# Nuos/jpgEnc

Hardware: AMD Instinct MI355X
Metric: MPixels/s encode (4K 4:2:0 Q=90) (higher is better)
Workload: dtype f64; 1 GPU; 3840x2160 4:2:0 Q90 full encode (RGB8 in HBM -> .jpg bytes in HBM), 3072 frames per GPU per step over 32 distinct inputs; width=3840, height=2160, quality=90, subsampling=4:2:0, distinct_inputs_per_gpu=32, parallelism=frames sharded over 1 GPU(s), no data-path collective, avg_jpeg_bytes=4581380

## Files before the change

jpgenc_amd/csrc/encoder.cpp:

```cpp
#include "encoder_impl.hpp"
#include "host_par.hpp"

#include <algorithm>
#include <array>
#include <condition_variable>
#include <cstdlib>
#include <cstdio>
#include <mutex>
#include <string>
#include <thread>

#include <sys/prctl.h>
#include <vector>

namespace jpge {

hipError_t wait_event(hipEvent_t e) {
    hipError_t r;
    while ((r = hipEventQuery(e)) == hipErrorNotReady) {
    }
    return r;
}
int wait_seq(const uint64_t* word, uint64_t seq, hipStream_t stream, int nap_us, const std::atomic<int>* queued,
             WaitGuess* guess, const std::function<bool()>* work) {
// ... 289 lines not shown
    if (mode) *mode = huff_mode_;
    if (specs && huff_mode_)
        for (int t = 0; t < 4; ++t) specs[t] = huff_specs_[t];
}

int Encoder::fixed_tables(Slot& s, bool& fresh) {
    const bool gray = s.g.gray();
    Slot::FixedKey k;
    k.gen = huff_gen_;
    k.w = s.img_w;
    k.h = s.img_h;
    k.restart = s.rst.mcus;
    k.samp = gray ? 0u : (s.g.yh << 4) | s.g.yv();
    std::memcpy(k.qy, s.qy, 64);
    std::memcpy(k.qc, s.qc, 64);
    s.symbols = 0;
    fresh = !(k == s.fixed);
    if (fresh) {
        s.fixed.gen = 0;
        std::memcpy(s.h_tab, huff_words_, kTabBytes);
        if (gray) std::memset(s.h_tab + 2 * 256, 0, 2 * 256 * sizeof(uint32_t));
        const HuffTable* tp[4] = {&huff_tabs_[0], &huff_tabs_[1], &huff_tabs_[2], &huff_tabs_[3]};
        const std::vector<uint8_t> hdr = gray ? jfif_headers_gray(s.img_w, s.img_h, s.qy, tp, s.rst.mcus)
                                              : jfif_headers(s.img_w, s.img_h, s.qy, s.qc, tp, s.rst.mcus,
                                                             (uint8_t)k.samp);
        if (hdr.size() > kHdrMax) return kErrInternal;
        std::memcpy(reinterpret_cast<uint8_t*>(s.h_tab) + kTabBytes, hdr.data(), hdr.size());
        s.hdr_len = hdr.size();
        s.fixed = k;
    }
    if (s.out_cap && s.out_cap < s.hdr_len + 2) return kErrNoSpace;
    return kOk;
}

size_t Encoder::max_jpeg_bytes(uint32_t w, uint32_t h) {
    size_t cap = 0;
    for (int mode : {420, 444, 422, 411}) {
        const Geometry g = geometry(w, h, mode);
        cap = std::max(cap, 2048 + (size_t)g.nblocks() * 2 * 209 + 16 + (size_t)g.nmcu() * 4);
    }
    return cap;
}

int Encoder::open(int device, std::unique_ptr<Encoder>& out, int lanes) {
    int n = 0;
    if (hipGetDeviceCount(&n) != hipSuccess || n <= 0) return kErrNoDevice;
    if (device < 0 || device >= n) return kErrNoDevice;
    JPGE_HIP(hipSetDevice(device));
    std::unique_ptr<Encoder> e(new Encoder());
    e->device_ = device;
    if (const char* ew = std::getenv("JPGE_ENTROPY_WGS")) e->entropy_wgs_ = (uint32_t)std::strtoul(ew, nullptr, 10);
    if (const char* sw = std::getenv("JPGE_STATS_WGS")) e->stats_wgs_ = (uint32_t)std::strtoul(sw, nullptr, 10);
    e->fdct_wgs_ = (uint32_t)env_int("JPGE_FDCT_WGS", 0, 0, 65536);
    e->stamps_file_ = std::getenv("JPGE_STAMPS_FILE");
    e->host_trace_file_ = std::getenv("JPGE_HOST_TRACE");
    e->cpu_prof_ = env_int("JPGE_CPU_PROF", 0, 0, 1) != 0;
    e->lat_prof_ = env_int("JPGE_LAT_PROF", 0, 0, 1) != 0;
    e->table_helper_ = env_int("JPGE_TABLE_HELPER", 1, 0, 1) != 0;
    e->gate_ = env_int("JPGE_GATE", 1, 0, 2);
    if (env_int("AMD_SERIALIZE_KERNEL", 0, 0, 3) != 0 || env_int("HIP_LAUNCH_BLOCKING", 0, 0, 1) != 0) e->gate_ = 0;
    if (const int us = env_int("JPGE_TEST_GATE_TIMEOUT_US", 0, 0, 1000000)) e->gate_ticks_ = 100ull * (uint64_t)us;
    e->gate_delay_us_ = env_int("JPGE_TEST_GATE_DELAY_US", 0, 0, 1000000);
    if (e->gate_ == 2) {
        int wv = 0;
        if (hipDeviceGetAttribute(&wv, hipDeviceAttributeCanUseStreamWaitValue, device) != hipSuccess || !wv) e->gate_ = 0;
        (void)hipGetLastError();
    }
    e->hist_nap_us_ = env_int("JPGE_HIST_NAP_US", e->hist_nap_us_, 0, 1000);
    e->lookahead_ = env_int("JPGE_LOOKAHEAD", e->lookahead_, 1, kMaxLookahead);
    e->drain_lag_ = env_int("JPGE_DRAIN_LAG", e->drain_lag_, 0, kMaxDrainLag);
    e->set_ = env_int("JPGE_SET", 0, 0, kMaxSet);
    e->nap_us_ = env_int("JPGE_NAP_US", e->nap_us_, 1, 1000);
    e->first_sleep_ = env_int("JPGE_FIRST_SLEEP", (int)(e->first_sleep_ * 100 + 0.5), 0, 95) / 100.0;
    const int nap = env_int("JPGE_NAP", -1, -1, 1);
    e->ext_place_ = env_int("JPGE_EXT_PLACE", -1, -1, 1);
    e->place_in_code_ = env_int("JPGE_PLACE_IN_CODE", 1, 0, 1) != 0;
    if (e->stamps_file_) {
        e->dbg_words_ = 4ull * 65536 * kStampSlots;
        JPGE_HIP(hipMalloc((void**)&e->d_dbg_, e->dbg_words_ * 8));
        JPGE_HIP(hipMemset(e->d_dbg_, 0, e->dbg_words_ * 8));
    }
    const int nlanes = e->stamps_file_ ? 1
                       : lanes > 0   ? std::min(lanes, kMaxLanes)
                                     : env_int("JPGE_LANES", 4, 1, kMaxLanes);
    e->nap_ = nap < 0 ? nlanes > 1 : nap != 0;
    const int nslots = e->lookahead_ + e->drain_lag_ + 1;
    const bool cumask = env_int("JPGE_CU_MASK_STREAMS", nlanes > 1 ? 1 : 0, 0, 1) != 0;
    std::vector<uint32_t> mask;
    if (cumask) {
        int ncu = 0;
        JPGE_HIP(hipDeviceGetAttribute(&ncu, hipDeviceAttributeMultiprocessorCount, device));
        mask.assign((size_t)(ncu + 31) / 32, 0xFFFFFFFFu);
        if (ncu % 32) mask.back() = (1u << (ncu % 32)) - 1u;
    }
    for (int l = 0; l < nlanes; ++l) {
        std::unique_ptr<Lane> ln(new Lane());
        ln->id = l;
        if (!cumask || hipExtStreamCreateWithCUMask(&ln->stream, (uint32_t)mask.size(), mask.data()) != hipSuccess) {
            (void)hipGetLastError();
            JPGE_HIP(hipStreamCreateWithFlags(&ln->stream, hipStreamNonBlocking));
        }
        JPGE_HIP(hipEventCreateWithFlags(&ln->done, hipEventDisableTiming));
        ln->guess_hist.frac = ln->guess_result.frac = e->first_sleep_;
        if (const int st = e->add_slots(*ln, nslots)) return st;
        if (l > 0) ln->start();
        e->lanes_.push_back(std::move(ln));
// ... 143 lines not shown
    a.imp_dst = imp ? reinterpret_cast<uint4*>(imp->d_tab) : nullptr;
    a.imp_n16 = imp ? (uint32_t)((kTabBytes + imp->hdr_len + 15) / 16) : 0u;
    a.dbg = d_dbg_;
    return a;
}

StatsArgs Encoder::stats_args(Slot& s) {
    const CtlLayout L(slot_layout(s).grid());
    StatsArgs st;
    st.coef = s.d_coef;
    st.g = s.g;
    st.hist.cnt = reinterpret_cast<uint32_t*>(s.d_ctl + L.cnt);
    st.hist.key = reinterpret_cast<uint64_t*>(s.d_ctl + L.key);
    st.seed = s.seed;
    st.rst = s.rst;
    st.key_y0 = s.key_y0;
    st.key_c0 = s.key_c0;
    st.key_ncb = s.key_ncb;
    st.seg = seg_layout(s.g, s.rst.mcus, entropy_wgs());
    st.recs = s.d_recs;
    st.tcount = s.d_tcount;
    st.wgs = stats_wgs();
    if (!stats_wgs_ && lanes_.size() > 1) {
        const uint32_t t = seg_tiles(st.seg);
        if (t < 3u * 384u) st.wgs = std::max(1u, (t + 2) / 3);
    }
    st.dbg = d_dbg_ ? d_dbg_ + 65536 * kStampSlots : nullptr;
    return st;
}

EntropyArgs Encoder::entropy_args(Slot& s) {
    const CtlLayout L(slot_layout(s).grid());
    EntropyArgs e;
    e.coef = s.d_coef;
    e.recs = s.d_recs;
    e.tcount = s.d_tcount;
    e.g = s.g;
    e.tables = s.d_tab;
    e.out = s.out_dev;
    e.hdr_len = s.hdr_len;
    e.out_cap = s.out_cap;
    e.rec = s.d_ctl + L.rec;
    e.place = reinterpret_cast<WgPlace*>(s.d_ctl + L.place);
    e.summary = reinterpret_cast<StripeSummary*>(s.d_ctl + L.summary);
    if (ext_place_ > 0 || (ext_place_ < 0 && lanes_.size() > 1)) {
        e.flags |= kExtPlace;
        if (place_in_code_ && !s.rst.mcus && slot_layout(s).grid() <= kPlaceInCodeMaxWgs)
            e.done = reinterpret_cast<uint32_t*>(s.d_ctl + L.done);
    }
    e.host_result = s.d_result_host;
    e.seq = s.seq;
    e.ubuf = s.d_ubuf;
    e.wgs = entropy_wgs_;
    e.seed = s.seed;
    e.rst = s.rst;
    e.seg = slot_layout(s);
    if (s.rst.mcus) {
        e.seg_index0 = s.rst.mcu0 / s.rst.mcus;
        e.seg_markers0 = e.seg_index0 > 0 ? 1u : 0u;
    }
    Slot::carry_export(e, nullptr);
    e.dbg = d_dbg_ ? d_dbg_ + 2 * 65536 * kStampSlots : nullptr;
    return e;
}

int Encoder::prep1(Slot& s, const FrameDesc& f, const uint8_t qy[64], const uint8_t qc[64], uint32_t flags,
                   Slot* imp, FdctArgs& a, StatsArgs& st) {
    if (!f.rgb || f.width == 0 || f.height == 0 || f.width > 65535 || f.height > 65535) return kErrArg;
    if (f.maxval < 1 || f.maxval > 255) return kErrRange;
    const bool gray = fmt_gray(f.fmt);
    const Geometry g = gray ? gray_geometry(f.width, f.height) : geometry(f.width, f.height, mode_);
    if (!fmt_valid(f.fmt) || (f.plane_stride && fmt_planes(f.fmt) == 1)) return kErrArg;
    if (fmt_yuv(f.fmt) && (f.maxval != 255 || (fmt_yuv420(f.fmt) && mode_ != 420))) return kErrArg;
    if (gray && f.maxval != 255) return kErrArg;
    if (fmt_yuv10(f.fmt) && (((uintptr_t)f.rgb | f.stride | f.plane_stride) & 1)) return kErrArg;
    if (gray) qc = qy;
    const size_t row = (size_t)fmt_row_bytes(f.fmt, f.width);
    const size_t stride = f.stride ? f.stride : row;
    if (stride < row) return kErrArg;
    const size_t planes = fmt_planes(f.fmt);
    const size_t plane_stride = f.plane_stride ? f.plane_stride : stride * f.height;
    const bool half = fmt_yuv420(f.fmt) || f.fmt == kFmtI422;
    const size_t dev_pitch = align_up(row, f.fmt == kFmtI420 || f.fmt == kFmtI422 || f.fmt == kFmtI010 ? 32 : 16);
    const size_t dev_plane = dev_pitch * f.height;
    const size_t crows = f.fmt == kFmtI422 ? f.height : chroma_dim(f.height),
                 crow = f.fmt == kFmtNv12 || f.fmt == kFmtP010 ? row : (size_t)fmt_bpp(f.fmt) * chroma_dim(f.width);
    const size_t cpitch = (size_t)fmt_chroma_pitch(f.fmt, stride), dev_cpitch = (size_t)fmt_chroma_pitch(f.fmt, dev_pitch);
    const size_t dev_bytes = half ? dev_plane + (planes - 1) * dev_cpitch * crows : planes * dev_plane;
    const bool dev_in = (flags & kFlagDeviceInput) != 0, dev_out = (flags & kFlagDeviceOutput) != 0;
    if (!k1_offsets_fit(f.fmt, g, dev_in ? stride : dev_pitch)) return kErrArg;
    const size_t in_bytes = dev_in ? 0 : dev_bytes;
    const size_t out_cap = dev_out ? 0 : max_jpeg_bytes(f.width, f.height);
    if (!tables_nonzero(qy, qc)) return kErrArg;
    const int st0 = ensure(s, g, in_bytes, out_cap);
    if (st0) return st0;
    if (!dev_in) {
        if (stride == dev_pitch && (planes == 1 || plane_stride == dev_plane))
            JPGE_HIP(hipMemcpyAsync(s.d_in, f.rgb, dev_bytes, hipMemcpyHostToDevice, s.stream));
        else if (half) {
            JPGE_HIP(hipMemcpy2DAsync(s.d_in, dev_pitch, f.rgb, stride, (size_t)fmt_bpp(f.fmt) * f.width, f.height, hipMemcpyHostToDevice,
                                      s.stream));
            for (size_t c = 0; c + 1 < planes; ++c)
                JPGE_HIP(hipMemcpy2DAsync(s.d_in + dev_plane + c * dev_cpitch * crows, dev_cpitch,
                                          f.rgb + plane_stride + c * cpitch * crows, cpitch, crow, crows,
                                          hipMemcpyHostToDevice, s.stream));
        } else
// ... 655 lines not shown
```

jpgenc_amd/csrc/encoder.hpp:

```cpp
#pragma once
#include <atomic>
#include <chrono>
#include <cstddef>
#include <cstdint>
#include <memory>
#include <functional>
#include <mutex>
#include <vector>

#include <hip/hip_runtime_api.h>

#include "host_io.hpp"
#include "huffman.hpp"
#include "kernels.hpp"
#include "planes.hpp"

namespace jpge {

constexpr uint32_t kFlagDeviceInput = 1u;
constexpr uint32_t kFlagDeviceOutput = 2u;
constexpr uint32_t kFlagCoefficients = 1u << 30;
constexpr uint32_t kFlagFixedTables = 1u << 29;

struct FrameDesc {
// ... 96 lines not shown
    int prep1(Slot& s, const FrameDesc& f, const uint8_t qy[64], const uint8_t qc[64], uint32_t flags, Slot* imp,
              FdctArgs& a, StatsArgs& st);
    int phase1_set(Slot* const* s, int n, const FdctArgs* a, const StatsArgs* st);
    int batch_set_size(const FrameDesc* fr, int n) const;
    int add_slots(Lane& ln, int count);
    int build_tables(Slot& s, bool parallel, TableHelper* helper = nullptr);
    int build_tables_from(Slot& s, const uint32_t* cnt, const uint64_t* first, bool parallel,
                          bool inverted = false,
                          TableHelper* helper = nullptr);
    FdctArgs fdct_args(Slot& s, int maxval, Slot* imp);
    StatsArgs stats_args(Slot& s);
    EntropyArgs entropy_args(Slot& s);
    EntropyArgs stripe_entropy_args(Slot& s);
    int import_tables_copy(Slot& s);
    int launch_entropy_phase(Slot& s, Slot* exp, bool lone = false, int parts = 3);
    int finish(Slot& s, FrameDesc& f, uint32_t flags, bool guess_wait = true, const std::function<bool()>* idle = nullptr);
    int export_hist(Slot& s);
    int await_call_end(Slot& s, uint32_t flags, int st);
    int run_lane(Lane& ln, FrameDesc* fr, int total, std::atomic<int>* next, int set, const uint8_t qy[64],
                 const uint8_t qc[64], uint32_t flags);
    int encode_fixed(FrameDesc& f, const uint8_t qy[64], const uint8_t qc[64], uint32_t flags);
    int fixed_tables(Slot& s, bool& fresh);

    int device_ = 0;
    int timing_every_ = 0;
    std::atomic<uint64_t> frame_counter_{0};
    std::atomic<uint64_t> seq_counter_{0};
    std::unique_ptr<TableHelper> helper_;
    bool table_helper_ = true;
    int gate_ = 1;
    uint32_t gate_count_ = 0;
    uint64_t gate_ticks_ = 100000000ull;
    int gate_delay_us_ = 0;
    std::atomic<uint64_t> gate_timeouts_{0};
  public:
    uint64_t gate_timeouts() const { return gate_timeouts_.load(std::memory_order_relaxed); }
  private:
    uint32_t entropy_wgs_ = 0;
    uint32_t stats_wgs_ = 0;
    uint32_t restart_mcus_ = 0;
    int mode_ = 420;
    int fmt_ = kFmtRgb8;
    int huff_mode_ = 0;
    HuffSpec huff_specs_[4] = {};
    HuffTable huff_tabs_[4];
    uint32_t huff_words_[4 * 256] = {};
    uint64_t huff_gen_ = 0;
    size_t plane_stride_ = 0;
    int yuv_preset_ = kYuvFull601;
    YuvXf yuv_xf_;
    uint32_t entropy_wgs() const {
        return entropy_wgs_ ? entropy_wgs_ : (lanes_.size() == 1 && set_ <= 1 ? 512u : 0u);
    }
    uint32_t stats_wgs() const { return stats_wgs_ ? stats_wgs_ : (lanes_.size() == 1 ? 768u : 384u); }
    SegLayout layout(const Geometry& g) const { return seg_layout(g, restart_mcus_, entropy_wgs()); }
    SegLayout slot_layout(const Slot& s) const;
    uint32_t fdct_wgs_ = 0;
    int lookahead_ = 2;
    int drain_lag_ = 1;
    int set_ = 0;
    int nap_us_ = 40;
    double first_sleep_ = 0.8;
    int ext_place_ = -1;
    bool place_in_code_ = true;
    bool nap_ = false;
    const char* host_trace_file_ = nullptr;
    bool cpu_prof_ = false;
    std::atomic<int64_t> cpu_ns_[6] = {};
    std::atomic<int64_t> cpu_frames_{0};
    std::atomic<int64_t> cpu_read_ns_{0}, cpu_build_ns_{0}, cpu_builds_{0}, cpu_part_ns_[3] = {};
    int hist_nap_us_ = 0;
    bool lat_prof_ = false;
    int64_t lat_ns_[8] = {}, lat_calls_ = 0;
    std::chrono::steady_clock::time_point lat_hist_seen_{};
    const char* stamps_file_ = nullptr;
    uint64_t* d_dbg_ = nullptr;
    size_t dbg_words_ = 0;
    void dump_stamps(const Slot& s);
    KernelTimes times_;
    std::mutex times_mu_;
    std::recursive_mutex call_mu_;
    std::vector<std::pair<void*, size_t>> scratch_;
    void* scratch(int i, size_t bytes);
  public:
    std::recursive_mutex& call_mutex() { return call_mu_; }
  private:
    std::mutex trace_mu_;
    std::vector<std::unique_ptr<Lane>> lanes_;
};

}
```

jpgenc_amd/csrc/entropy.hip:

```cpp
#include "device_common.hpp"

namespace jpge {
namespace {
using namespace dev;

constexpr int kK3Groups = 2;
constexpr int kK3Wpe = 7;
constexpr int kK3Blocks = kEntropyTile;
constexpr int kK3Threads = kK3Blocks * kPartsPerBlock;
constexpr int kK3Waves = kK3Threads / 64;
constexpr int kMaxTiles = kEntropyMaxTilesPerWg;
constexpr int kTcntSlots = kMaxTiles * kRecSub;
constexpr int kStageWords = kK3Blocks * kStageBytesPerBlock / 4 + 4;
constexpr int kWin = 32;
constexpr int kWinWords = kWin / 4;
static_assert(kWinWords == 8 && kEntropyRegionBytes % 16 == 0, "pack loads a window as two aligned uint4");
constexpr int kPackStoreAux = 16;
constexpr int kPackStoreNt = 2;
constexpr int kChunk = kK3Threads * kWin;

struct alignas(16) WgRecord {
    uint32_t ff[8];
    uint32_t bits;
    uint32_t edge;
// ... 434 lines not shown
                const uint32_t b = (uint32_t)((p + al) & 7);
                c[al] += r[b];
                if (b && k > 0) c[al] += split_bits((R(k - 1)[kRecEdge] >> 8) & 0xFF, r[kRecEdge], b) == 0xFF;
            }
            p += r[kRecBits];
        }
    }
#pragma unroll
    for (int al = 0; al < 8; ++al) {
        uint32_t v = c[al];
#pragma unroll
        for (int d = 32; d >= 1; d >>= 1) v += __shfl_xor(v, d);
        if (lane == 0 && v) atomicAdd(&tot8[al], v);
    }
    __syncthreads();
    if (tid == 0) {
        StripeSummary sm{};
        sm.bits = total;
#pragma unroll
        for (int al = 0; al < 8; ++al) sm.ff[al] = tot8[al];
        sm.head = R(0)[kRecEdge] & 0xFF;
        sm.tail = (R(G - 1)[kRecEdge] >> 8) & 0xFF;
        *a.summary = sm;
    }
}

__device__ void place_all(const EntropyArgs& a, uint32_t G, uint32_t* wsum, int tid) {
    const RecView R{a.rec, G};
    scan_records<kK3Waves>(a, R, wsum, tid, [&](uint32_t k, uint64_t p, uint64_t q, uint32_t o) {
        a.place[k] = make_place(R, k, p, q, o, a);
    });
}

constexpr int kPlaceThreads = 256;
constexpr uint32_t kPlaceSmallMaxWgs = 4096;
__global__ __launch_bounds__(kPlaceThreads) void entropy_place_kernel(EntropyArgs a, uint32_t G) {
    __shared__ uint32_t wsum[2 * (kPlaceThreads / 64)];
    const RecView R{a.rec, G};
    scan_records<kPlaceThreads / 64>(a, R, wsum, threadIdx.x, [&](uint32_t k, uint64_t p, uint64_t q, uint32_t o) {
        a.place[k] = make_place(R, k, p, q, o, a);
    });
}
hipError_t launch_place(const EntropyArgs& b, uint32_t G, hipStream_t s) {
    if (!b.rst.mcus && G <= kPlaceSmallMaxWgs && kPlaceThreads < kScanThreads)
        hipLaunchKernelGGL(entropy_place_kernel, dim3(1), dim3(kPlaceThreads), 0, s, b, G);
    else
        hipLaunchKernelGGL(entropy_scan_kernel, dim3(1), dim3(kScanThreads), 0, s, b, G, 0);
    return hipGetLastError();
}

struct PackLds {
    uint8_t ob[2 * kChunk + 8];
    uint32_t wsum[2 * kK3Waves];
    uint64_t P, Q;
    uint32_t Lb, ftotal, split, fill, seg;
};

template <int kN>
__global__ __launch_bounds__(kK3Threads) void entropy_pack_kernel(FrameSet<EntropyArgs, kN> fs) {
    __shared__ PackLds S;
    const uint32_t set_f = set_member<kN>(fs.wg0, fs.n, blockIdx.x);
    const EntropyArgs& a = fs.a[set_f];
    const int tid = threadIdx.x, lane = tid & 63, wv = tid >> 6;
    const uint32_t wg = blockIdx.x - fs.wg0[set_f], G = fs.wg0[set_f + 1] - fs.wg0[set_f];
    const bool last = wg == G - 1;
    const bool eoi = last && (a.flags & kStripeLast);
    const WgTiles wt = wg_tiles(a.seg, wg);
    const bool fills = a.rst.mcus ? wt.last : eoi;
    JPGE_STAMP(0);
    const bool wthru = a.pack_done != nullptr;
    const __amdgpu_buffer_rsrc_t out_rs = __builtin_amdgcn_make_buffer_rsrc(
        a.out, 0, (int)(a.out_cap < 0x7FFFFFF0ull ? a.out_cap : 0x7FFFFFF0ull), 0x00020000);
    auto out_byte = [&](uint64_t i, uint32_t v) {
        __builtin_amdgcn_raw_buffer_store_b8((uint8_t)v, out_rs, (uint32_t)i, 0, kPackStoreAux);
    };
    if (wg == 0 && (a.flags & kStripeFirst)) {
        const uint8_t* hdr = reinterpret_cast<const uint8_t*>(a.tables + 1024);
        for (uint32_t i = tid; i < a.hdr_len; i += kK3Threads) out_byte(i, hdr[i]);
    }

    const RecView R{a.rec, G};
    if (a.flags & kExtPlace) {
        if (tid == 0) {
            const WgPlace w = a.place[wg];
            S.P = w.P;
            S.Q = w.Q;
            S.ftotal = w.ftotal;
            S.split = w.split;
            S.fill = w.fill;
            S.seg = w.seg;
            S.Lb = R(wg)[kRecBits];
        }
    } else {
        scan_records<kK3Waves>(a, R, S.wsum, tid, [&](uint32_t k, uint64_t p, uint64_t q, uint32_t o) {
            if (k != wg) return;
            const WgPlace w = make_place(R, k, p, q, o, a);
            S.P = w.P;
            S.Q = w.Q;
            S.ftotal = w.ftotal;
            S.split = w.split;
            S.fill = w.fill;
            S.seg = 0;
            S.Lb = R(k)[kRecBits];
        });
    }
    __syncthreads();
    JPGE_STAMP(1);

    const uint64_t P = S.P;
    const uint32_t b = (uint32_t)(P & 7), Lb = S.Lb, ftotal = S.ftotal;
    const uint32_t nc = (b + Lb) >> 3;
    const uint32_t eb = (b + Lb) & 7;
    const uint32_t n_own = nc + ((fills && eb) ? 1u : 0u);
    const uint32_t markers = a.rst.mcus ? S.seg + a.seg_markers0 : 0u;
    const uint64_t D0 = a.hdr_len + a.out_base + (P >> 3) + S.Q + 2ull * markers;
    const uint64_t ntot = (uint64_t)n_own + ftotal + (eoi ? 2u : 0u);
    const bool fits = D0 + ntot <= a.out_cap;
    if (fits && wt.first && markers && tid == 0) {
        uint8_t* const m = a.out + D0 - 2;
        const __amdgpu_buffer_rsrc_t mrs = __builtin_amdgcn_make_buffer_rsrc(m, 0, 2, 0x00020000);
        __builtin_amdgcn_raw_buffer_store_b8((uint8_t)0xFF, mrs, 0, 0, kPackStoreAux);
        __builtin_amdgcn_raw_buffer_store_b8((uint8_t)(0xD0 + ((a.seg_index0 + S.seg - 1) & 7)), mrs, 1, 0,
                                             kPackStoreAux);
    }
    const uint32_t split = S.split, fill = S.fill;
    const uint32_t* R32 = reinterpret_cast<const uint32_t*>(a.ubuf + (uint64_t)wg * kEntropyRegionBytes);
    const uint32_t nwr = (Lb + 31) >> 5;
    auto rword = [&](int64_t m) -> uint32_t {
        return (m >= 0 && m < (int64_t)nwr) ? __builtin_bswap32(R32[m]) : 0u;
    };
    uint64_t d = D0;
    for (uint32_t c = 0; fits && c < n_own; c += kChunk) {
        const uint32_t j0 = c + kWin * tid;
        const uint32_t jhi = min(j0 + kWin, n_own);
        uint32_t y[kWinWords];
        uint32_t cff = 0;
        if (j0 < jhi) {
            const uint32_t w0 = j0 / 4;
            const uint4* R4 = reinterpret_cast<const uint4*>(R32 + w0);
            const uint4 lo = R4[0], hi = R4[1];
            const uint32_t raw[kWinWords] = {lo.x, lo.y, lo.z, lo.w, hi.x, hi.y, hi.z, hi.w};
            uint32_t prev = rword((int64_t)w0 - 1);
#pragma unroll
            for (int m = 0; m < kWinWords; ++m) {
                const uint32_t cur = w0 + m < nwr ? __builtin_bswap32(raw[m]) : 0u;
                y[m] = __builtin_amdgcn_alignbit(prev, cur, b);
                prev = cur;
            }
            if (j0 == 0 && b) y[0] = (y[0] & 0x00FFFFFFu) | (split << 24);
            if (fills && eb && n_own - 1 < j0 + kWin) {
                const uint32_t q = n_own - 1 - j0, sh = 24 - 8 * (q & 3);
#pragma unroll
                for (int m = 0; m < kWinWords; ++m)
                    if ((int)(q >> 2) == m) y[m] = (y[m] & ~(0xFFu << sh)) | (fill << sh);
            }
#pragma unroll
            for (int m = 0; m < kWinWords; ++m) {
                const int n = min((int)(jhi - j0) - 4 * m, 4);
                if (n > 0) cff += __builtin_popcount(ff_bytes(y[m]) & byte_range(0, n));
            }
        }
        uint32_t chunk_ff;
        const uint32_t excl = block_scan<kK3Waves, uint32_t, uint32_t, false, false>(cff, S.wsum, lane, wv, chunk_ff);
        const uint32_t cend = min(c + (uint32_t)kChunk, n_own);
        const uint32_t align = (uint32_t)(d & 3);
        if (j0 < jhi) {
            uint32_t o = align + (j0 - c) + excl;
            if (cff == 0 && jhi - j0 == (uint32_t)kWin) {
                uint32_t z[kWinWords];
#pragma unroll
                for (int m = 0; m < kWinWords; ++m) z[m] = __builtin_bswap32(y[m]);
                uint32_t* ob32 = reinterpret_cast<uint32_t*>(S.ob);
                const uint32_t r = o & 3u;
                if (r == 0) {
#pragma unroll
                    for (int m = 0; m < kWinWords; ++m) ob32[(o >> 2) + m] = z[m];
                } else {
#pragma unroll
                    for (uint32_t q = 0; q < 3; ++q)
                        if (q < 4u - r) S.ob[o + q] = (uint8_t)(z[0] >> (8 * q));
                    const uint32_t wb = (o + 4u - r) >> 2;
#pragma unroll
                    for (int m = 0; m < kWinWords - 1; ++m) ob32[wb + m] = __builtin_amdgcn_alignbyte(z[m + 1], z[m], 4u - r);
#pragma unroll
                    for (uint32_t q = 0; q < 3; ++q)
                        if (q < r) S.ob[o + kWin - r + q] = (uint8_t)(z[kWinWords - 1] >> (8 * (4u - r + q)));
                }
            } else {
#pragma unroll
                for (int q = 0; q < kWin; ++q) {
                    if (j0 + q < jhi) {
                        const uint8_t v = (uint8_t)(y[q >> 2] >> (24 - 8 * (q & 3)));
                        S.ob[o++] = v;
                        if (v == 0xFF) S.ob[o++] = 0;
                    }
                }
            }
        }
        const uint32_t clen = (cend - c) + chunk_ff;
        __syncthreads();
        uint8_t* gout = a.out + (d - align);
        const uint32_t nw = (align + clen + 3) / 4;
        const __amdgpu_buffer_rsrc_t ors = __builtin_amdgcn_make_buffer_rsrc(gout, 0, (int)(4 * nw), 0x00020000);
        for (uint32_t w = tid; w < nw; w += kK3Threads) {
            const uint32_t s = 4 * w, e = s + 4;
            if (s >= align && e <= align + clen) {
                const uint32_t v = *reinterpret_cast<const uint32_t*>(S.ob + s);
                if (wthru) __builtin_amdgcn_raw_buffer_store_b32(v, ors, s, 0, kPackStoreAux);
                else __builtin_amdgcn_raw_buffer_store_b32(v, ors, s, 0, kPackStoreNt);
            } else {
                for (uint32_t q = max(s, align); q < min(e, align + clen); ++q)
                    __builtin_amdgcn_raw_buffer_store_b8(S.ob[q], ors, q, 0, kPackStoreAux);
            }
        }
        d += clen;
        if (c + kChunk < n_own) __syncthreads();
    }
    if (last && tid == 0) {
        uint64_t len = 0;
        if (fits) {
            if (eoi) {
                uint8_t* const m = a.out + d;
                const __amdgpu_buffer_rsrc_t mrs = __builtin_amdgcn_make_buffer_rsrc(m, 0, 2, 0x00020000);
                __builtin_amdgcn_raw_buffer_store_b8((uint8_t)0xFF, mrs, 0, 0, kPackStoreAux);
                __builtin_amdgcn_raw_buffer_store_b8((uint8_t)0xD9, mrs, 1, 0, kPackStoreAux);
                d += 2;
            }
            len = d;
        }
        if (a.pack_done) {
            __hip_atomic_store(reinterpret_cast<uint64_t*>(a.pack_done + 2), len, __ATOMIC_RELAXED, __HIP_MEMORY_SCOPE_AGENT);
            __hip_atomic_store(a.pack_done + 4, fits ? 0u : 4u, __ATOMIC_RELAXED, __HIP_MEMORY_SCOPE_AGENT);
        } else if (a.host_result) {
            __hip_atomic_store(&a.host_result[0], len, __ATOMIC_RELAXED, __HIP_MEMORY_SCOPE_SYSTEM);
            __hip_atomic_store(&a.host_result[1], fits ? 0ull : 4ull, __ATOMIC_RELAXED, __HIP_MEMORY_SCOPE_SYSTEM);
            __hip_atomic_store(&a.host_result[3], a.seq, __ATOMIC_RELEASE, __HIP_MEMORY_SCOPE_SYSTEM);
        }
    }
    if (a.pack_done) {
        vm_drain();
        __syncthreads();
        if (tid == 0 && atomicAdd(a.pack_done, 1u) == G - 1 && a.host_result) {
            __builtin_amdgcn_fence(__ATOMIC_ACQUIRE, "agent");
            const uint64_t len =
                __hip_atomic_load(reinterpret_cast<const uint64_t*>(a.pack_done + 2), __ATOMIC_RELAXED, __HIP_MEMORY_SCOPE_AGENT);
            const uint32_t nospace = __hip_atomic_load(a.pack_done + 4, __ATOMIC_RELAXED, __HIP_MEMORY_SCOPE_AGENT);
            __hip_atomic_store(a.pack_done, 0u, __ATOMIC_RELAXED, __HIP_MEMORY_SCOPE_AGENT);
            __hip_atomic_store(&a.host_result[0], len, __ATOMIC_RELAXED, __HIP_MEMORY_SCOPE_SYSTEM);
            __hip_atomic_store(&a.host_result[1], (uint64_t)nospace, __ATOMIC_RELAXED, __HIP_MEMORY_SCOPE_SYSTEM);
            __hip_atomic_store(&a.host_result[3], a.seq, __ATOMIC_RELEASE, __HIP_MEMORY_SCOPE_SYSTEM);
        }
    }
    JPGE_STAMP(2);
}

}

SegLayout seg_layout(const Geometry& g, uint32_t restart_mcus, uint32_t wgs_override) {
    SegLayout L;
    const uint32_t nb = g.nblocks();
    const uint32_t want = wgs_override ? wgs_override : 384u;
    const uint64_t S = (uint64_t)g.bpm * restart_mcus;
    if (!restart_mcus || S >= nb) {
        const uint32_t nt = (nb + kK3Blocks - 1) / kK3Blocks;
        uint32_t G = 1;
        if (nt > 1) {
            const uint32_t lo = (nt + kMaxTiles - 1) / kMaxTiles, hi = nt;
            const uint32_t w = wgs_override ? want : (nt < 2u * want ? (nt + 1) / 2 : want);
            G = w < lo ? lo : (w > hi ? hi : w);
        }
        L.nseg = 1;
        L.sblk = L.lblk = nb;
        L.tps = L.ltps = nt;
        L.wps = L.lwps = G;
        return L;
    }
    L.nseg = (uint32_t)((nb + S - 1) / S);
    L.sblk = (uint32_t)S;
    L.lblk = nb - (L.nseg - 1) * L.sblk;
    const uint32_t per_seg = (want + L.nseg - 1) / L.nseg;
    auto part = [&](uint32_t blocks, uint32_t& tps, uint32_t& wps) {
        tps = (blocks + kK3Blocks - 1) / kK3Blocks;
        const uint32_t lo = (tps + kMaxTiles - 1) / kMaxTiles;
        wps = per_seg < lo ? lo : (per_seg > tps ? tps : per_seg);
    };
    part(L.sblk, L.tps, L.wps);
    part(L.lblk, L.ltps, L.lwps);
    return L;
}

constexpr uint32_t kGateThreads = 512;
__global__ __launch_bounds__(kGateThreads) void gate_copy_kernel(const uint32_t* gate, uint32_t value, const uint4* src,
                                                                 uint4* dst, uint32_t n16, uint64_t* fail,
                                                                 uint64_t timeout_ticks) {
    __shared__ uint32_t open;
    if (threadIdx.x == 0) {
        const uint64_t t0 = __builtin_amdgcn_s_memrealtime();
        uint32_t o = 1;
        while (__hip_atomic_load(gate, __ATOMIC_ACQUIRE, __HIP_MEMORY_SCOPE_SYSTEM) != value) {
            __builtin_amdgcn_s_sleep(4);
            if (__builtin_amdgcn_s_memrealtime() - t0 > timeout_ticks) {
                o = 0;
                break;
            }
        }
        open = o;
    }
    __syncthreads();
    if (!open) {
        if (threadIdx.x == 0) __hip_atomic_store(fail, 1ull, __ATOMIC_RELAXED, __HIP_MEMORY_SCOPE_SYSTEM);
        return;
    }
    __atomic_thread_fence(__ATOMIC_ACQUIRE);
    for (uint32_t i = threadIdx.x; i < n16; i += kGateThreads) dst[i] = src[i];
}

hipError_t launch_gate_copy(const uint32_t* gate, uint32_t value, const void* src, void* dst, uint32_t n16,
                            uint64_t* fail, uint64_t timeout_ticks, hipStream_t s) {
    hipLaunchKernelGGL(gate_copy_kernel, dim3(1), dim3(kGateThreads), 0, s, gate, value,
                       reinterpret_cast<const uint4*>(src), reinterpret_cast<uint4*>(dst), n16, fail, timeout_ticks);
    return hipGetLastError();
}

hipError_t launch_entropy(const EntropyArgs& a, hipStream_t s, const KTimer* tcode, const KTimer* tpack) {
    const hipError_t e = launch_entropy_code(a, s, tcode);
    return e != hipSuccess ? e : launch_entropy_pack(a, s, tpack);
}

hipError_t launch_entropy_code(const EntropyArgs& a, hipStream_t s, const KTimer* tcode) {
    const uint32_t G = a.seg.grid();
    return launch_timed(tcode, entropy_code_kernel<1>, dim3(G), dim3(kK3Threads), s, frame_set<1>(&a, 1, G));
}

hipError_t launch_entropy_pack(const EntropyArgs& a, hipStream_t s, const KTimer* tpack) {
    const uint32_t G = a.seg.grid();
    hipError_t e = hipSuccess;
    EntropyArgs b = a;
    b.dbg = a.dbg ? a.dbg + 65536 * kStampSlots : nullptr;
    if (a.done) {
        if (!a.place || a.rst.mcus || G > kPlaceInCodeMaxWgs) return hipErrorInvalidValue;
        b.flags |= kExtPlace;
    } else if (G > kInlineScanMaxWgs || (a.flags & kExtPlace) || a.rst.mcus) {
        if (!a.place) return hipErrorInvalidValue;
        b.flags |= kExtPlace;
        if ((e = launch_place(b, G, s)) != hipSuccess) return e;
    }
    return launch_timed(tpack, entropy_pack_kernel<1>, dim3(G), dim3(kK3Threads), s, frame_set<1>(&b, 1, G));
}

hipError_t launch_entropy_set(const EntropyArgs* a, int n, hipStream_t s, const KTimer* tcode, const KTimer* tpack) {
    if (n < 1 || n > kMaxSet) return hipErrorInvalidValue;
    const uint32_t G = a[0].seg.grid();
    FrameSet<EntropyArgs> fs = frame_set(a, n, G);
    for (int f = 0; f < n; ++f) {
        const EntropyArgs& m = a[f];
        if (m.seg.grid() != G || !m.done || !m.place || m.rst.mcus || G > kPlaceInCodeMaxWgs) return hipErrorInvalidValue;
    }
    hipError_t e = launch_timed(tcode, entropy_code_kernel<kMaxSet>, dim3(G * n), dim3(kK3Threads), s, fs);
    if (e != hipSuccess) return e;
    for (int f = 0; f < n; ++f) {
        fs.a[f].flags |= kExtPlace;
        fs.a[f].dbg = a[f].dbg ? a[f].dbg + 65536 * kStampSlots : nullptr;
    }
    return launch_timed(tpack, entropy_pack_kernel<kMaxSet>, dim3(G * n), dim3(kK3Threads), s, fs);
}

hipError_t launch_entropy_code_summary(const EntropyArgs& a, hipStream_t s) {
    const uint32_t G = a.seg.grid();
    if (!a.summary) return hipErrorInvalidValue;
    hipLaunchKernelGGL(entropy_code_kernel<1>, dim3(G), dim3(kK3Threads), 0, s, frame_set<1>(&a, 1, G));
    hipError_t e = hipGetLastError();
    if (e != hipSuccess) return e;
    hipLaunchKernelGGL(entropy_scan_kernel, dim3(1), dim3(kScanThreads), 0, s, a, G, a.rst.mcus ? 0 : 1);
    return hipGetLastError();
}

hipError_t launch_entropy_place_pack(const EntropyArgs& a, hipStream_t s) {
    const uint32_t G = a.seg.grid();
    if (!a.place) return hipErrorInvalidValue;
    EntropyArgs b = a;
    b.flags |= kExtPlace;
    if (!a.rst.mcus) {
        const hipError_t e = launch_place(b, G, s);
        if (e != hipSuccess) return e;
    }
    hipLaunchKernelGGL(entropy_pack_kernel<1>, dim3(G), dim3(kK3Threads), 0, s, frame_set<1>(&b, 1, G));
    return hipGetLastError();
}

}
```

jpgenc_amd/csrc/kernels.hpp:

```cpp
#pragma once
#include <cstdint>

#include <hip/hip_runtime_api.h>

#if defined(__HIPCC__)
#define JPGE_HD __host__ __device__
#else
#define JPGE_HD
#endif

namespace jpge {

constexpr uint32_t kFiltS420m = 0, kFiltS420lm = 1, kFiltS420 = 2;
struct Geometry {
    uint32_t width = 0, height = 0;
    uint32_t mw = 0, mh = 0;
    uint32_t bpm = 6;
    uint32_t yh = 2;
    uint32_t cfilt = kFiltS420m;
    JPGE_HD uint32_t nmcu() const { return mw * mh; }
    JPGE_HD uint32_t nblocks() const { return nmcu() * bpm; }
    JPGE_HD bool gray() const { return bpm == 1; }
    JPGE_HD uint32_t ny() const { return gray() ? 1u : bpm - 2; }
    JPGE_HD uint32_t yv() const { return ny() / yh; }
// ... 162 lines not shown
    uint64_t Q;
    uint32_t ftotal;
    uint32_t split;
    uint32_t fill;
    uint32_t seg;
};

struct StripeSummary {
    uint64_t bits;
    uint32_t ff[8];
    uint32_t head;
    uint32_t tail;
    uint32_t restart;
    uint32_t pad;
};

constexpr uint32_t kStripeFirst = 1u;
constexpr uint32_t kStripeLast = 2u;
constexpr uint32_t kExtPlace = 4u;

struct EntropyArgs {
    const int16_t* coef;
    const uint16_t* recs;
    const uint32_t* tcount;
    Geometry g;
    const uint32_t* tables;
    uint8_t* out;
    uint64_t hdr_len;
    uint64_t out_cap;
    uint8_t* ubuf;
    uint8_t* rec;
    uint32_t* done = nullptr;
    uint32_t* pack_done = nullptr;
    uint64_t* host_result;
    uint64_t seq;
    HistPtrs exp_hist;
    uint32_t* exp_cnt;
    uint64_t* exp_key;
    uint64_t* exp_seq;
    uint64_t exp_seqv;
    uint32_t wgs;
    DcSeed seed;
    uint64_t p_ext = 0, q_ext = 0;
    uint32_t head_split = 0;
    uint32_t flags = kStripeFirst | kStripeLast;
    WgPlace* place = nullptr;
    StripeSummary* summary = nullptr;
    Restart rst;
    SegLayout seg;
    uint32_t seg_markers0 = 0;
    uint32_t seg_index0 = 0;
    uint64_t out_base = 0;
    uint64_t* dbg;
};

JPGE_HD inline uint32_t seg_tiles(const SegLayout& L) { return (L.nseg - 1) * L.tps + L.ltps; }
JPGE_HD inline void seg_tile(const SegLayout& L, uint32_t gt, uint64_t& b0, uint32_t& nb) {
    uint32_t seg, i, tps, nbs;
    if (gt < (L.nseg - 1) * L.tps) {
        seg = gt / L.tps; i = gt % L.tps; tps = L.tps; nbs = L.sblk;
    } else {
        seg = L.nseg - 1; i = gt - seg * L.tps; tps = L.ltps; nbs = L.lblk;
    }
    b0 = (uint64_t)seg * L.sblk + (uint64_t)i * nbs / tps;
    nb = (uint32_t)((uint64_t)(i + 1) * nbs / tps - (uint64_t)i * nbs / tps);
}
JPGE_HD inline void sub_tile(const SegLayout& L, uint32_t s, uint64_t& b0, uint32_t& nb) {
    uint64_t tb;
    uint32_t tn;
    seg_tile(L, s / kRecSub, tb, tn);
    const uint32_t j = s % kRecSub;
    b0 = tb + j * tn / kRecSub;
    nb = (j + 1) * tn / kRecSub - j * tn / kRecSub;
}

inline uint32_t entropy_tiles(const Geometry& g) {
    return (g.nblocks() + kEntropyTile - 1) / kEntropyTile;
}
constexpr uint64_t kEntropyRegionBytes = (uint64_t)kEntropyMaxTilesPerWg * kEntropyTile * kStageBytesPerBlock + 128;

struct KTimer {
    hipEvent_t start = nullptr, stop = nullptr;
};

constexpr int kMaxSet = 4;
template <typename A, int N = kMaxSet>
struct FrameSet {
    A a[N];
    uint32_t wg0[N + 1];
    uint32_t n;
};
JPGE_HD inline uint32_t set_member_rolled(const uint32_t* wg0, uint32_t n, uint32_t b) {
    uint32_t f = 0;
    for (uint32_t i = 1; i < n; ++i) f += b >= wg0[i] ? 1u : 0u;
    return f;
}
template <int N>
JPGE_HD inline uint32_t set_member(const uint32_t* wg0, uint32_t n, uint32_t b) {
    uint32_t f = 0;
    for (int i = 1; i < N; ++i) f += (i < (int)n && b >= wg0[i]) ? 1u : 0u;
    return f;
}
template <int N = kMaxSet, typename A>
inline FrameSet<A, N> frame_set(const A* a, int n, uint32_t grid_each) {
    FrameSet<A, N> s{};
    s.n = (uint32_t)n;
    for (int f = 0; f < n; ++f) {
// ... 47 lines not shown
```

Baseline: 247,400 MPix/s.

## Let pack workgroups span several regions and prefetch next window via buffer loads

Lets each entropy pack workgroup handle up to pack_span consecutive code regions, with the pack grid shrunk to match. It also software-pipelines the bitstream window loads: the next chunk's 128-bit buffer loads are issued before the current chunk is processed, replacing direct global reads. Uniform values are forced to scalar registers with readfirstlane, and LDS-only barriers replace __syncthreads. The default span stays 1, so the main gain is meant to come from prefetching that hides load latency, at the cost of more live registers and more complex control flow.

Measured after the change: 248,100 MPix/s (median of 2 runs). Within noise of the previous version (+0.3%).

```diff
diff --git a/jpgenc_amd/csrc/encoder.cpp b/jpgenc_amd/csrc/encoder.cpp
--- a/jpgenc_amd/csrc/encoder.cpp
+++ b/jpgenc_amd/csrc/encoder.cpp
@@ -365,6 +365,7 @@
     if (const char* ew = std::getenv("JPGE_ENTROPY_WGS")) e->entropy_wgs_ = (uint32_t)std::strtoul(ew, nullptr, 10);
     if (const char* sw = std::getenv("JPGE_STATS_WGS")) e->stats_wgs_ = (uint32_t)std::strtoul(sw, nullptr, 10);
     e->fdct_wgs_ = (uint32_t)env_int("JPGE_FDCT_WGS", 0, 0, 65536);
+    e->pack_span_ = env_int("JPGE_PACK_SPAN", 0, 0, (int)kMaxPackSpan);
     e->stamps_file_ = std::getenv("JPGE_STAMPS_FILE");
     e->host_trace_file_ = std::getenv("JPGE_HOST_TRACE");
     e->cpu_prof_ = env_int("JPGE_CPU_PROF", 0, 0, 1) != 0;
@@ -614,6 +615,7 @@
     e.seq = s.seq;
     e.ubuf = s.d_ubuf;
     e.wgs = entropy_wgs_;
+    e.pack_span = pack_span();
     e.seed = s.seed;
     e.rst = s.rst;
     e.seg = slot_layout(s);
diff --git a/jpgenc_amd/csrc/encoder.hpp b/jpgenc_amd/csrc/encoder.hpp
--- a/jpgenc_amd/csrc/encoder.hpp
+++ b/jpgenc_amd/csrc/encoder.hpp
@@ -172,6 +172,9 @@
     uint32_t entropy_wgs() const {
         return entropy_wgs_ ? entropy_wgs_ : (lanes_.size() == 1 && set_ <= 1 ? 512u : 0u);
     }
+    static constexpr uint32_t kPipelinePackSpan = 1;
+    int pack_span_ = 0;
+    uint32_t pack_span() const { return pack_span_ ? (uint32_t)pack_span_ : (lanes_.size() > 1 ? kPipelinePackSpan : 1u); }
     uint32_t stats_wgs() const { return stats_wgs_ ? stats_wgs_ : (lanes_.size() == 1 ? 768u : 384u); }
     SegLayout layout(const Geometry& g) const { return seg_layout(g, restart_mcus_, entropy_wgs()); }
     SegLayout slot_layout(const Slot& s) const;
diff --git a/jpgenc_amd/csrc/entropy.hip b/jpgenc_amd/csrc/entropy.hip
--- a/jpgenc_amd/csrc/entropy.hip
+++ b/jpgenc_amd/csrc/entropy.hip
@@ -510,9 +510,12 @@
 struct PackLds {
     uint8_t ob[2 * kChunk + 8];
     uint32_t wsum[2 * kK3Waves];
-    uint64_t P, Q;
-    uint32_t Lb, ftotal, split, fill, seg;
+    WgPlace pl[kMaxPackSpan];
+    uint32_t Lb[kMaxPackSpan];
 };
+
+__device__ __forceinline__ uint32_t uni(uint32_t v) { return __builtin_amdgcn_readfirstlane(v); }
+__device__ __forceinline__ uint64_t uni(uint64_t v) { return ((uint64_t)uni((uint32_t)(v >> 32)) << 32) | uni((uint32_t)v); }
 
 template <int kN>
 __global__ __launch_bounds__(kK3Threads) void entropy_pack_kernel(FrameSet<EntropyArgs, kN> fs) {
@@ -520,11 +523,25 @@
     const uint32_t set_f = set_member<kN>(fs.wg0, fs.n, blockIdx.x);
     const EntropyArgs& a = fs.a[set_f];
     const int tid = threadIdx.x, lane = tid & 63, wv = tid >> 6;
-    const uint32_t wg = blockIdx.x - fs.wg0[set_f], G = fs.wg0[set_f + 1] - fs.wg0[set_f];
-    const bool last = wg == G - 1;
+    const uint32_t wg = blockIdx.x - fs.wg0[set_f], Gp = fs.wg0[set_f + 1] - fs.wg0[set_f];
+    const uint32_t G = a.seg.grid(), span = pack_span(a);
+    const uint32_t r0 = wg * span, ns = min(span, G - r0);
+    const bool last = r0 + ns == G;
     const bool eoi = last && (a.flags & kStripeLast);
-    const WgTiles wt = wg_tiles(a.seg, wg);
-    const bool fills = a.rst.mcus ? wt.last : eoi;
+    auto win_load = [&](uint32_t r, bool ok, uint32_t c, uint32_t Lb, uint4& lo, uint4& hi, uint32_t& pw) {
+        const uint32_t nbytes = min((((Lb + 31u) >> 5) * 4u + (uint32_t)kWin - 1u) & ~((uint32_t)kWin - 1u),
+                                    (uint32_t)kEntropyRegionBytes);
+        const __amdgpu_buffer_rsrc_t rs = __builtin_amdgcn_make_buffer_rsrc(
+            a.ubuf + (uint64_t)(ok ? r : r0) * kEntropyRegionBytes, 0, (int)nbytes, 0x00020000);
+        const uint32_t off = ok ? c + kWin * (uint32_t)tid : 0x80000000u;
+        lo = as_u4(__builtin_amdgcn_raw_buffer_load_b128(rs, off, 0, 0));
+        hi = as_u4(__builtin_amdgcn_raw_buffer_load_b128(rs, off + 16u, 0, 0));
+        pw = __builtin_amdgcn_raw_buffer_load_b32(rs, off ? off - 4u : 0x80000000u, 0, 0);
+    };
+    uint4 nlo, nhi;
+    uint32_t npw;
+    const RecView R{a.rec, G};
+    win_load(r0, true, 0, uni(R(r0)[kRecBits]), nlo, nhi, npw);
     JPGE_STAMP(0);
     const bool wthru = a.pack_done != nullptr;
     const __amdgpu_buffer_rsrc_t out_rs = __builtin_amdgcn_make_buffer_rsrc(
@@ -532,73 +549,76 @@
     auto out_byte = [&](uint64_t i, uint32_t v) {
         __builtin_amdgcn_raw_buffer_store_b8((uint8_t)v, out_rs, (uint32_t)i, 0, kPackStoreAux);
     };
-    if (wg == 0 && (a.flags & kStripeFirst)) {
+    if (r0 == 0 && (a.flags & kStripeFirst)) {
         const uint8_t* hdr = reinterpret_cast<const uint8_t*>(a.tables + 1024);
         for (uint32_t i = tid; i < a.hdr_len; i += kK3Threads) out_byte(i, hdr[i]);
     }
 
-    const RecView R{a.rec, G};
     if (a.flags & kExtPlace) {
-        if (tid == 0) {
-            const WgPlace w = a.place[wg];
-            S.P = w.P;
-            S.Q = w.Q;
-            S.ftotal = w.ftotal;
-            S.split = w.split;
-            S.fill = w.fill;
-            S.seg = w.seg;
-            S.Lb = R(wg)[kRecBits];
+        if ((uint32_t)tid < ns) {
+            S.pl[tid] = a.place[r0 + tid];
+            S.Lb[tid] = R(r0 + tid)[kRecBits];
         }
     } else {
         scan_records<kK3Waves>(a, R, S.wsum, tid, [&](uint32_t k, uint64_t p, uint64_t q, uint32_t o) {
-            if (k != wg) return;
-            const WgPlace w = make_place(R, k, p, q, o, a);
-            S.P = w.P;
-            S.Q = w.Q;
-            S.ftotal = w.ftotal;
-            S.split = w.split;
-            S.fill = w.fill;
-            S.seg = 0;
-            S.Lb = R(k)[kRecBits];
+            if (k - r0 >= ns) return;
+            S.pl[k - r0] = make_place(R, k, p, q, o, a);
+            S.Lb[k - r0] = R(k)[kRecBits];
         });
     }
-    __syncthreads();
+    lds_barrier();
     JPGE_STAMP(1);
 
-    const uint64_t P = S.P;
-    const uint32_t b = (uint32_t)(P & 7), Lb = S.Lb, ftotal = S.ftotal;
-    const uint32_t nc = (b + Lb) >> 3;
-    const uint32_t eb = (b + Lb) & 7;
-    const uint32_t n_own = nc + ((fills && eb) ? 1u : 0u);
-    const uint32_t markers = a.rst.mcus ? S.seg + a.seg_markers0 : 0u;
-    const uint64_t D0 = a.hdr_len + a.out_base + (P >> 3) + S.Q + 2ull * markers;
-    const uint64_t ntot = (uint64_t)n_own + ftotal + (eoi ? 2u : 0u);
-    const bool fits = D0 + ntot <= a.out_cap;
-    if (fits && wt.first && markers && tid == 0) {
-        uint8_t* const m = a.out + D0 - 2;
-        const __amdgpu_buffer_rsrc_t mrs = __builtin_amdgcn_make_buffer_rsrc(m, 0, 2, 0x00020000);
-        __builtin_amdgcn_raw_buffer_store_b8((uint8_t)0xFF, mrs, 0, 0, kPackStoreAux);
-        __builtin_amdgcn_raw_buffer_store_b8((uint8_t)(0xD0 + ((a.seg_index0 + S.seg - 1) & 7)), mrs, 1, 0,
-                                             kPackStoreAux);
-    }
-    const uint32_t split = S.split, fill = S.fill;
-    const uint32_t* R32 = reinterpret_cast<const uint32_t*>(a.ubuf + (uint64_t)wg * kEntropyRegionBytes);
-    const uint32_t nwr = (Lb + 31) >> 5;
-    auto rword = [&](int64_t m) -> uint32_t {
-        return (m >= 0 && m < (int64_t)nwr) ? __builtin_bswap32(R32[m]) : 0u;
-    };
-    uint64_t d = D0;
-    for (uint32_t c = 0; fits && c < n_own; c += kChunk) {
+    uint64_t d = 0;
+    uint32_t fits = 1;
+    uint32_t dn = 0;
+    for (uint32_t k = 0, c = 0; k < ns;) {
+        const uint32_t r = r0 + k;
+        const uint64_t P = uni(S.pl[k].P);
+        const uint32_t b = (uint32_t)(P & 7), Lb = uni(S.Lb[k]), ftotal = uni(S.pl[k].ftotal);
+        const uint32_t seg = uni(S.pl[k].seg), split = uni(S.pl[k].split), fill = uni(S.pl[k].fill);
+        const uint32_t ends = r == G - 1 && (a.flags & kStripeLast) ? 1u : 0u;
+        uint32_t seg_first = 0, fills = ends;
+        if (a.rst.mcus) {
+            const WgTiles wt = wg_tiles(a.seg, r);
+            seg_first = wt.first ? 1u : 0u;
+            fills = wt.last ? 1u : 0u;
+        }
+        const uint32_t nc = (b + Lb) >> 3;
+        const uint32_t eb = (b + Lb) & 7;
+        const uint32_t n_own = nc + ((fills && eb) ? 1u : 0u);
+        const uint32_t nwr = (Lb + 31) >> 5;
+        const uint32_t markers = a.rst.mcus ? seg + a.seg_markers0 : 0u;
+        const uint64_t D0 = a.hdr_len + a.out_base + (P >> 3) + uni(S.pl[k].Q) + 2ull * markers;
+        const uint64_t ntot = (uint64_t)n_own + ftotal + 2u * ends;
+        fits = D0 + ntot <= a.out_cap ? 1u : 0u;
+        if (c == 0) dn = 0;
+        d = D0 + dn;
+        if (c == 0 && fits && seg_first && markers && tid == 0) {
+            uint8_t* const m = a.out + D0 - 2;
+            const __amdgpu_buffer_rsrc_t mrs = __builtin_amdgcn_make_buffer_rsrc(m, 0, 2, 0x00020000);
+            __builtin_amdgcn_raw_buffer_store_b8((uint8_t)0xFF, mrs, 0, 0, kPackStoreAux);
+            __builtin_amdgcn_raw_buffer_store_b8((uint8_t)(0xD0 + ((a.seg_index0 + seg - 1) & 7)), mrs, 1, 0,
+                                                 kPackStoreAux);
+        }
+        const uint4 lo = nlo, hi = nhi;
+        const uint32_t pw = npw;
+        const uint32_t more = fits && c + kChunk < n_own ? 1u : 0u;
+        const uint32_t nk = k + 1u - more, ncx = more ? c + kChunk : 0u;
+        win_load(r0 + nk, nk < ns, ncx, uni(S.Lb[nk < ns ? nk : k]), nlo, nhi, npw);
+        if (!(fits && c < n_own)) {
+            k = nk;
+            c = ncx;
+            continue;
+        }
         const uint32_t j0 = c + kWin * tid;
         const uint32_t jhi = min(j0 + kWin, n_own);
         uint32_t y[kWinWords];
         uint32_t cff = 0;
         if (j0 < jhi) {
             const uint32_t w0 = j0 / 4;
-            const uint4* R4 = reinterpret_cast<const uint4*>(R32 + w0);
-            const uint4 lo = R4[0], hi = R4[1];
             const uint32_t raw[kWinWords] = {lo.x, lo.y, lo.z, lo.w, hi.x, hi.y, hi.z, hi.w};
-            uint32_t prev = rword((int64_t)w0 - 1);
+            uint32_t prev = w0 - 1u < nwr ? __builtin_bswap32(pw) : 0u;
 #pragma unroll
             for (int m = 0; m < kWinWords; ++m) {
                 const uint32_t cur = w0 + m < nwr ? __builtin_bswap32(raw[m]) : 0u;
@@ -619,7 +639,7 @@
             }
         }
         uint32_t chunk_ff;
-        const uint32_t excl = block_scan<kK3Waves, uint32_t, uint32_t, false, false>(cff, S.wsum, lane, wv, chunk_ff);
+        const uint32_t excl = block_scan<kK3Waves, uint32_t, uint32_t, true, false>(cff, S.wsum, lane, wv, chunk_ff);
         const uint32_t cend = min(c + (uint32_t)kChunk, n_own);
         const uint32_t align = (uint32_t)(d & 3);
         if (j0 < jhi) {
@@ -655,8 +675,10 @@
                 }
             }
         }
-        const uint32_t clen = (cend - c) + chunk_ff;
-        __syncthreads();
+        const uint32_t clen = (cend - c) + uni(chunk_ff);
+        lds_barrier();
+        asm volatile("" : "+v"(nlo.x), "+v"(nlo.y), "+v"(nlo.z), "+v"(nlo.w), "+v"(nhi.x), "+v"(nhi.y), "+v"(nhi.z),
+                     "+v"(nhi.w), "+v"(npw));
         uint8_t* gout = a.out + (d - align);
         const uint32_t nw = (align + clen + 3) / 4;
         const __amdgpu_buffer_rsrc_t ors = __builtin_amdgcn_make_buffer_rsrc(gout, 0, (int)(4 * nw), 0x00020000);
@@ -672,7 +694,10 @@
             }
         }
         d += clen;
-        if (c + kChunk < n_own) __syncthreads();
+        dn += clen;
+        if (nk < ns) lds_barrier();
+        k = nk;
+        c = ncx;
     }
     if (last && tid == 0) {
         uint64_t len = 0;
@@ -698,7 +723,7 @@
     if (a.pack_done) {
         vm_drain();
         __syncthreads();
-        if (tid == 0 && atomicAdd(a.pack_done, 1u) == G - 1 && a.host_result) {
+        if (tid == 0 && atomicAdd(a.pack_done, 1u) == Gp - 1 && a.host_result) {
             __builtin_amdgcn_fence(__ATOMIC_ACQUIRE, "agent");
             const uint64_t len =
                 __hip_atomic_load(reinterpret_cast<const uint64_t*>(a.pack_done + 2), __ATOMIC_RELAXED, __HIP_MEMORY_SCOPE_AGENT);
@@ -803,7 +828,8 @@
         b.flags |= kExtPlace;
         if ((e = launch_place(b, G, s)) != hipSuccess) return e;
     }
-    return launch_timed(tpack, entropy_pack_kernel<1>, dim3(G), dim3(kK3Threads), s, frame_set<1>(&b, 1, G));
+    const uint32_t Gp = pack_grid(G, pack_span(b));
+    return launch_timed(tpack, entropy_pack_kernel<1>, dim3(Gp), dim3(kK3Threads), s, frame_set<1>(&b, 1, Gp));
 }
 
 hipError_t launch_entropy_set(const EntropyArgs* a, int n, hipStream_t s, const KTimer* tcode, const KTimer* tpack) {
@@ -816,11 +842,14 @@
     }
     hipError_t e = launch_timed(tcode, entropy_code_kernel<kMaxSet>, dim3(G * n), dim3(kK3Threads), s, fs);
     if (e != hipSuccess) return e;
+    const uint32_t span = pack_span(a[0]), Gp = pack_grid(G, span);
+    FrameSet<EntropyArgs> ps = frame_set(a, n, Gp);
     for (int f = 0; f < n; ++f) {
-        fs.a[f].flags |= kExtPlace;
-        fs.a[f].dbg = a[f].dbg ? a[f].dbg + 65536 * kStampSlots : nullptr;
-    }
-    return launch_timed(tpack, entropy_pack_kernel<kMaxSet>, dim3(G * n), dim3(kK3Threads), s, fs);
+        ps.a[f].flags |= kExtPlace;
+        ps.a[f].pack_span = span;
+        ps.a[f].dbg = a[f].dbg ? a[f].dbg + 65536 * kStampSlots : nullptr;
+    }
+    return launch_timed(tpack, entropy_pack_kernel<kMaxSet>, dim3(Gp * n), dim3(kK3Threads), s, ps);
 }
 
 hipError_t launch_entropy_code_summary(const EntropyArgs& a, hipStream_t s) {
@@ -842,7 +871,8 @@
         const hipError_t e = launch_place(b, G, s);
         if (e != hipSuccess) return e;
     }
-    hipLaunchKernelGGL(entropy_pack_kernel<1>, dim3(G), dim3(kK3Threads), 0, s, frame_set<1>(&b, 1, G));
+    const uint32_t Gp = pack_grid(G, pack_span(b));
+    hipLaunchKernelGGL(entropy_pack_kernel<1>, dim3(Gp), dim3(kK3Threads), 0, s, frame_set<1>(&b, 1, Gp));
     return hipGetLastError();
 }
 
diff --git a/jpgenc_amd/csrc/kernels.hpp b/jpgenc_amd/csrc/kernels.hpp
--- a/jpgenc_amd/csrc/kernels.hpp
+++ b/jpgenc_amd/csrc/kernels.hpp
@@ -238,7 +238,14 @@
     uint32_t seg_index0 = 0;
     uint64_t out_base = 0;
     uint64_t* dbg;
-};
+    uint32_t pack_span = 1;
+};
+
+constexpr uint32_t kMaxPackSpan = 8;
+JPGE_HD inline uint32_t pack_span(const EntropyArgs& a) {
+    return a.pack_span < 1u ? 1u : (a.pack_span > kMaxPackSpan ? kMaxPackSpan : a.pack_span);
+}
+JPGE_HD inline uint32_t pack_grid(uint32_t G, uint32_t span) { return (G + span - 1) / span; }
 
 JPGE_HD inline uint32_t seg_tiles(const SegLayout& L) { return (L.nseg - 1) * L.tps + L.ltps; }
 JPGE_HD inline void seg_tile(const SegLayout& L, uint32_t gt, uint64_t& b0, uint32_t& nb) {
```
